# ihmcrobotics/mecano

Hardware: AMD Instinct MI355X
Metric: robot-configs/sec (RNEA+ABA), 30-DoF humanoid batch=4096 (higher is better)
Workload: dtype f64; 1 GPU; 30-DoF humanoid (SixDoF pelvis + 24 revolute), RNEA and ABA of every configuration per step, fp64, AoS [B][n] state; entry_point=mh_rnea_aba_f64, batch_per_gpu=4096, global_batch=4096, nq=31, nv=30, bodies=25, parallelism=dp1 (batch sharded, no data-path collective), kernel_variant=topo:b5c1e26c784c54fa, model_seed=43, state_seed=2342

## Files before the change

mecano_amd/csrc/mh_api.hip:

```cpp
#include "../../include/mecano_hip.h"
#include "mh_dfs_kernels.h"
#include "mh_split_kernels.h"
#include "mh_gravity_kernels.h"
#include "mh_response_kernels.h"
#include "mh_minv_kernels.h"
#include "mh_rnea_deriv_kernels.h"
#include "mh_params_kernels.h"

#include <dlfcn.h>
#include <spawn.h>
#include <sys/wait.h>
#include <unistd.h>
#include <cerrno>
extern char **environ;
#include <unistd.h>

#include <algorithm>
#include <functional>
#include <array>
#include <cmath>
#include <cstdarg>
#include <cstdio>
#include <cstdlib>
#include <cstring>
// ... 122 lines not shown
      T::operator=(v);
      return *this;
   }
};
}

struct SpecLib
{
   void *handle = nullptr;
   int (*launch)(int algo, int flags, const void *args, int grid, void *stream) = nullptr;
   long (*lds_bytes)(int algo, int flags, int nq, int nv) = nullptr;
   int (*aba_slots)(void) = nullptr;
   int (*supports)(int algo, int flags) = nullptr;
   int (*launch_fused)(int flags, const void *args, int waves, void *stream) = nullptr;
   long (*fused_lds_bytes)(int nq, int nv) = nullptr;
   int (*launch_crba)(int flags, const void *args, int grid, void *stream) = nullptr;
   int (*crba_packed)(int flags) = nullptr;
   int (*split_usable)(void) = nullptr;
   long (*split_lds_bytes)(int algo, int flags, int nq, int nv) = nullptr;
   int (*launch_split)(int algo, int flags, const void *args, int groups, void *stream) = nullptr;
   int (*crba_split_usable)(void) = nullptr;
   int (*launch_crba_split)(const void *args, int groups, int lanes_per_group, void *stream) = nullptr;
   int (*launch_rnea_crba)(const void *args, int rnea_groups, int crba_groups, int lanes_per_group, void *stream) = nullptr;
   long (*rnea_crba_lds_bytes)(int lanes_per_group, int nq, int nv) = nullptr;
   int (*launch_coriolis)(int flags, const void *args, int grid, void *stream) = nullptr;
   int (*launch_centroidal)(int flags, const void *args, int grid, void *stream) = nullptr;
   int (*launch_coriolis_parts)(int flags, const void *args, int grid, int parts, void *stream) = nullptr;
   int (*launch_centroidal_parts)(int flags, const void *args, int grid, int parts, void *stream) = nullptr;
   unsigned long long (*abi)(void) = nullptr;
   const char *(*sources_hash)(void) = nullptr;
   int (*zv_usable)(void) = nullptr;
   long (*zv_lds_bytes)(int nq, int nv) = nullptr;
   int (*launch_zv)(int flags, const void *args, void *taup, int *sync_flags, int *error, int epoch, int jobs, int same_l2, unsigned wait_ticks, void *stream) = nullptr;
   int (*zv_self_signal)(void) = nullptr;
   int (*zvb_usable)(void) = nullptr;
   int (*zvb_cs_rows)(void) = nullptr;
   long (*zvb_lds_bytes)(int which, int nq, int nv) = nullptr;
   int (*launch_zvb)(int flags, const void *args, void *taup, void *cs, long cs_stride, int groups, int which, void *stream) = nullptr;
   int (*zvf_usable)(void) = nullptr;
   int (*zvf_pair_usable)(void) = nullptr;
   int (*launch_zvf)(int flags, const void *args, int groups, void *stream) = nullptr;
   int (*launch_rnea_ahead)(int flags, const void *args, int groups, void *stream) = nullptr;
};
enum : int
{
   SPEC_IO_LDS = 1,
   SPEC_IDENT = 2,
   SPEC_ST_LDS = 4,
   SPEC_BODIES = 16,
   SPEC_OCC3 = 32
};

struct mh_model
{
   int n = 0, nq = 0, nv = 0, n_slots = 0;
   SpecLib spec;
   std::string topo_key;
   int device = 0;
   int cu_count = 256;
   std::vector<int> meta, dof_map, cfg_map;
   std::vector<int> engine_of;
   std::vector<double> consts;
   int *d_meta = nullptr, *d_dof = nullptr, *d_cfg = nullptr, *d_prog = nullptr;
   std::vector<int> prog;
   std::vector<int> prog_seq;
   int *d_prog_seq = nullptr;
// ... 278 lines not shown
}
std::mutex g_error_words_mutex;
std::vector<int *> g_error_words;
mh_status zv_check_error(mh_model *m)
{
   if (m->zv_error_host && *(volatile int *)m->zv_error_host != 0)
   {
      *(volatile int *)m->zv_error_host = 0;
      return fail(MH_ERR_HIP, "a bias-split forward dynamics launch gave up waiting for its bias rows (the accelerations of those configurations were written as NaN)");
   }
   return MH_OK;
}
mh_status check_all_error_words()
{
   std::lock_guard<std::mutex> lock(g_error_words_mutex);
   bool any = false;
   for (int *w : g_error_words)
      if (*(volatile int *)w != 0)
      {
         *(volatile int *)w = 0;
         any = true;
      }
   if (any)
      return fail(MH_ERR_HIP, "a bias-split forward dynamics launch gave up waiting for its bias rows (the accelerations of those configurations were written as NaN)");
   return MH_OK;
}
bool zv_self_signalling(const mh_model *m) { return m->ident_maps && m->spec.zv_self_signal && m->spec.zv_self_signal() != 0; }
mh_status zv_prepare(mh_model *m, int64_t B, hipStream_t stream)
{
   const size_t groups = (size_t)groups_of(B);
   mh_status st = ensure_bytes(m->zv_tau, groups * 64 * m->nv * sizeof(double));
   if (st != MH_OK)
      return st;
   if (zv_self_signalling(m) && m->zv_cols.bytes < groups * 64 * m->nv * sizeof(double))
   {
      st = ensure_bytes(m->zv_cols, std::max<size_t>(groups, 128) * 64 * m->nv * sizeof(double));
      if (st != MH_OK)
         return st;
      HIP_TRY(hipMemsetD32Async((hipDeviceptr_t)m->zv_cols.ptr, 0x7ff4a5a5, m->zv_cols.bytes / 4, stream));
   }
   if (m->zv_flags.bytes < groups * mh::ZV_SYNC_STRIDE * sizeof(int))
   {
      st = ensure_bytes(m->zv_flags, std::max<size_t>(groups, 1024) * mh::ZV_SYNC_STRIDE * sizeof(int));
      if (st != MH_OK)
         return st;
      HIP_TRY(hipMemsetAsync(m->zv_flags.ptr, 0, m->zv_flags.bytes, stream));
      m->zv_epoch = 0;
   }
   if (!m->zv_error_host)
   {
      HIP_TRY(hipHostMalloc((void **)&m->zv_error_host, 2 * sizeof(int), hipHostMallocMapped));
      m->zv_error_host[0] = m->zv_error_host[1] = 0;
      HIP_TRY(hipHostGetDevicePointer((void **)&m->zv_error_dev, m->zv_error_host, 0));
      std::lock_guard<std::mutex> lock(g_error_words_mutex);
      g_error_words.push_back(m->zv_error_host);
   }
   return MH_OK;
}
mh_status zv_launch(mh_model *m, mh::Args<double> &A, int jobs, hipStream_t stream, bool &done)
{
   done = false;
   mh_status st = zv_prepare(m, A.B, stream);
   if (st != MH_OK)
      return st;
   if (m->zv_epoch == 0x7fffffff)
   {
      HIP_TRY(hipDeviceSynchronize());
      HIP_TRY(hipMemsetAsync(m->zv_flags.ptr, 0, m->zv_flags.bytes, stream));
      m->zv_epoch = 0;
// ... 1140 lines not shown
      dir = e;
   std::string path = dir + "/libmecano_hip_topo_" + P.key + ".so";
   void *h = dlopen(path.c_str(), RTLD_NOW | RTLD_LOCAL);
   if (!h)
   {
      path = dir + "/libmecano_hip_topo_" + P.key + ".min.so";
      h = dlopen(path.c_str(), RTLD_NOW | RTLD_LOCAL);
   }
   if (!h)
      return;
   auto f_n = (int (*)(void))dlsym(h, "mh_spec_n");
   auto f_p = (const int *(*)(void))dlsym(h, "mh_spec_parents");
   auto f_t = (const int *(*)(void))dlsym(h, "mh_spec_types");
   SpecLib s;
   s.handle = h;
   s.launch = (decltype(s.launch))dlsym(h, "mh_spec_launch");
   s.lds_bytes = (decltype(s.lds_bytes))dlsym(h, "mh_spec_lds_bytes");
   s.aba_slots = (decltype(s.aba_slots))dlsym(h, "mh_spec_aba_slots");
   s.supports = (decltype(s.supports))dlsym(h, "mh_spec_supports");
   s.launch_fused = (decltype(s.launch_fused))dlsym(h, "mh_spec_launch_fused");
   s.fused_lds_bytes = (decltype(s.fused_lds_bytes))dlsym(h, "mh_spec_fused_lds_bytes");
   s.launch_crba = (decltype(s.launch_crba))dlsym(h, "mh_spec_launch_crba");
   s.crba_packed = (decltype(s.crba_packed))dlsym(h, "mh_spec_crba_packed");
   s.split_usable = (decltype(s.split_usable))dlsym(h, "mh_spec_split_usable");
   s.split_lds_bytes = (decltype(s.split_lds_bytes))dlsym(h, "mh_spec_split_lds_bytes");
   s.launch_split = (decltype(s.launch_split))dlsym(h, "mh_spec_launch_split");
   s.crba_split_usable = (decltype(s.crba_split_usable))dlsym(h, "mh_spec_crba_split_usable");
   s.launch_crba_split = (decltype(s.launch_crba_split))dlsym(h, "mh_spec_launch_crba_split");
   s.launch_rnea_crba = (decltype(s.launch_rnea_crba))dlsym(h, "mh_spec_launch_rnea_crba");
   s.zv_usable = (decltype(s.zv_usable))dlsym(h, "mh_spec_zv_usable");
   s.zv_lds_bytes = (decltype(s.zv_lds_bytes))dlsym(h, "mh_spec_zv_lds_bytes");
   s.launch_zv = (decltype(s.launch_zv))dlsym(h, "mh_spec_launch_zv");
   s.zv_self_signal = (decltype(s.zv_self_signal))dlsym(h, "mh_spec_zv_self_signal");
   s.zvb_usable = (decltype(s.zvb_usable))dlsym(h, "mh_spec_zvb_usable");
   s.zvb_cs_rows = (decltype(s.zvb_cs_rows))dlsym(h, "mh_spec_zvb_cs_rows");
   s.zvb_lds_bytes = (decltype(s.zvb_lds_bytes))dlsym(h, "mh_spec_zvb_lds_bytes");
   s.launch_zvb = (decltype(s.launch_zvb))dlsym(h, "mh_spec_launch_zvb");
   s.zvf_usable = (decltype(s.zvf_usable))dlsym(h, "mh_spec_zvf_usable");
   s.zvf_pair_usable = (decltype(s.zvf_pair_usable))dlsym(h, "mh_spec_zvf_pair_usable");
   s.launch_zvf = (decltype(s.launch_zvf))dlsym(h, "mh_spec_launch_zvf");
   s.launch_rnea_ahead = (decltype(s.launch_rnea_ahead))dlsym(h, "mh_spec_launch_rnea_ahead");
   s.rnea_crba_lds_bytes = (decltype(s.rnea_crba_lds_bytes))dlsym(h, "mh_spec_rnea_crba_lds_bytes");
   s.launch_coriolis = (decltype(s.launch_coriolis))dlsym(h, "mh_spec_launch_coriolis");
   s.launch_centroidal = (decltype(s.launch_centroidal))dlsym(h, "mh_spec_launch_centroidal");
   s.launch_coriolis_parts = (decltype(s.launch_coriolis_parts))dlsym(h, "mh_spec_launch_coriolis_parts");
   s.launch_centroidal_parts = (decltype(s.launch_centroidal_parts))dlsym(h, "mh_spec_launch_centroidal_parts");
   s.abi = (decltype(s.abi))dlsym(h, "mh_spec_abi");
   if (!s.abi || s.abi() != mh::spec_abi_stamp())
   {
      char note[256];
      snprintf(note, sizeof note, "generic (code object %s refused: built against another library version, ABI stamp %016llx, this library %016llx)",
               path.c_str(), s.abi ? s.abi() : 0ull, mh::spec_abi_stamp());
      m->variant = note;
      dlclose(h);
      return;
   }
   s.sources_hash = (decltype(s.sources_hash))dlsym(h, "mh_spec_sources_hash");
   if (!s.sources_hash || strcmp(s.sources_hash(), MH_STR_(MH_SPEC_SOURCES_HASH)) != 0)
   {
      char note[320];
      snprintf(note, sizeof note, "generic (code object %s refused: built from other kernel sources or flags, source hash %s, this library expects %s)",
               path.c_str(), s.sources_hash ? s.sources_hash() : "(none)", MH_STR_(MH_SPEC_SOURCES_HASH));
      m->variant = note;
      dlclose(h);
      return;
   }
// ... 2488 lines not shown
```

mecano_amd/csrc/mh_spec.hip:

```cpp
#include "mh_spec_kernels.h"
#include "mh_zv_kernels.h"

#include <algorithm>
#include <atomic>
#include <cstdlib>
#include <type_traits>

#ifndef MH_SPEC_PART
#define MH_SPEC_PART 0
#endif
#ifndef MH_TOPO_N
#error "MH_TOPO_N / MH_TOPO_PARENTS / MH_TOPO_TYPES must be defined"
#endif

namespace
{
struct TP
{
   static constexpr int N = MH_TOPO_N;
   static constexpr int parent[N] = {MH_TOPO_PARENTS};
   static constexpr int type[N] = {MH_TOPO_TYPES};
};
constexpr int kParents[TP::N] = {MH_TOPO_PARENTS};
constexpr int kTypes[TP::N] = {MH_TOPO_TYPES};
// ... 193 lines not shown
#else
      if constexpr (SPL::usable())
      {
         if (id && io && (algo == 0 || algo == 1))
         {
            static LdsAttr attr0, attr1;
            const size_t lds = (size_t)split_lds_bytes(algo, F_IO_LDS, A.m.nq, A.m.nv);
            if (algo == 0)
               return (int)launch_lds(&mh::spec_split_kernel<TP, double, 0, true, true, true>, A, groups, lds, attr0, s);
            return (int)launch_lds(&mh::spec_split_kernel<TP, double, 1, true, true, true>, A, groups, lds, attr1, s);
         }
      }
      return (int)hipErrorNotSupported;
#endif
   }
   if (id && io)
      return (int)go_split_algo<true, true>(algo, A, groups, s, occ3);
#ifdef MH_SPEC_MINIMAL
   return (int)hipErrorNotSupported;
#else
   if (id)
      return (int)go_split_algo<true, false>(algo, A, groups, s, occ3);
   if (io)
      return (int)go_split_algo<false, true>(algo, A, groups, s, occ3);
   return (int)go_split_algo<false, false>(algo, A, groups, s, occ3);
#endif
}
#endif
#if MH_SPEC_PART != 1
long mh_spec_zv_lds_bytes(int nq, int nv)
{
   if constexpr (!SPL::usable())
      return 0;
   const long inertia = (long)(SPL::n_limbs() * mh::ZV_XW + SPL::ZV_TRUNK_SLOTS + nq + 2 * nv) * 64 * (long)sizeof(double);
   return std::max(inertia, split_lds_bytes(0, F_IO_LDS, nq, nv) + (long)mh::zv_bias_extra_rows<TP>() * 64 * (long)sizeof(double));
}
int mh_spec_zv_usable(void) { return SPL::usable() ? 1 : 0; }
int mh_spec_zv_self_signal(void) { return MH_ZV_TWO_STAGE && MH_ZV_SELF_SIGNAL ? 1 : 0; }
#ifdef MH_ZV_PROBE
int mh_spec_zv_probe_read(void *dst, size_t bytes) { return (int)hipMemcpyFromSymbol(dst, HIP_SYMBOL(mh::zv_probe), bytes); }
int mh_spec_zv_probe_body_read(void *dst, size_t bytes) { return (int)hipMemcpyFromSymbol(dst, HIP_SYMBOL(mh::zv_probe_body), bytes); }
#endif
int mh_spec_launch_zv(int flags, const void *args, void *taup, int *sync_flags, int *error, int epoch, int jobs, int same_l2, unsigned wait_ticks, void *stream)
{
   if constexpr (SPL::usable())
   {
      const mh::Args<double> &A = *(const mh::Args<double> *)args;
      if (!(flags & F_IO_LDS) || (jobs != 2 && jobs != 3))
         return (int)hipErrorNotSupported;
      const size_t lds = (size_t)mh_spec_zv_lds_bytes(A.m.nq, A.m.nv);
      if (lds > 160 * 1024)
         return (int)hipErrorNotSupported;
      const long groups = (A.B + 63) / 64, padded = (groups + 7) / 8 * 8;
      const mh::ZvSync sy{sync_flags, error, epoch, jobs, same_l2 ? 1 : 0, wait_ticks};
      hipStream_t s = (hipStream_t)stream;
      if (A.q_next && (!(flags & F_IDENT) || jobs != 2 || !MH_ZV_TWO_STAGE))
         return (int)hipErrorNotSupported;
      if ((flags & F_IDENT) && A.q_next)
      {
         static LdsAttr attr_step;
         auto kern = &mh::spec_zv_kernel<TP, double, true, true>;
         if (const hipError_t e = ensure_lds_attr(reinterpret_cast<const void *>(kern), lds, attr_step); e != hipSuccess)
            return (int)e;
         hipLaunchKernelGGL(kern, dim3((unsigned)(padded * jobs)), dim3(256), lds, s, A.q, A.qd, A.in3b, A.B, jobs, A, (double *)taup, sy);
         return (int)hipGetLastError();
      }
      if (flags & F_IDENT)
      {
         static LdsAttr attr;
         auto kern = &mh::spec_zv_kernel<TP, double, true>;
         if (const hipError_t e = ensure_lds_attr(reinterpret_cast<const void *>(kern), lds, attr); e != hipSuccess)
// ... 355 lines not shown
```

mecano_amd/csrc/mh_zv_kernels.h:

```cpp
#pragma once
#include "mh_spec_kernels.h"

namespace mh
{
template <class TP>
struct ZvStore
{
   static constexpr int REG_SLOTS = Split<TP>::zv_reg_slots();
   static constexpr int kind(int j) { return Split<TP>::is_trunk(j) ? ST_LDS_KIND : ST_REG_KIND; }
   static constexpr int index(int j) { return Split<TP>::is_trunk(j) ? Split<TP>::zv_trunk_slot(j) : Split<TP>::zv_reg_slot(j); }
   static constexpr bool shared(int j) { return !Split<TP>::is_trunk(j); }
};
template <class TP>
struct ZvbStore
{
   using S = Split<TP>;
   static constexpr bool root_in_regs(int j) { return S::staged() && j == S::root(); }
   static constexpr int REG_SLOTS = S::zv_reg_slots() + (S::staged() ? Tree<TP>::zv_slots_of(S::root() < 0 ? 0 : S::root(), true) : 0);
   static constexpr int trunk_slot(int j)
   {
      int s = 0;
      for (int i = 0; i < j; i++)
         s += S::is_trunk(i) && !root_in_regs(i) ? Tree<TP>::zv_slots_of(i, false) : 0;
      return s;
// ... 477 lines not shown
            const SV<T> pa = pA + SV<T>{u * sa, u * sl};
            up = force_up(TYPE, jx, Xb, pa);
         }
      }
      else if constexpr (TYPE == JT_SIXDOF)
      {
         SV<T> tau;
         if constexpr (CX::csmode == 3)
            tau = SV<T>{V3<T>{zvf_tau_get1<TP, J, 0, CX, T>(cx), zvf_tau_get1<TP, J, 1, CX, T>(cx), zvf_tau_get1<TP, J, 2, CX, T>(cx)},
                        V3<T>{zvf_tau_get1<TP, J, 3, CX, T>(cx), zvf_tau_get1<TP, J, 4, CX, T>(cx), zvf_tau_get1<TP, J, 5, CX, T>(cx)}};
         else
            tau = spec_vec<TYPE, DO, 1, CX, T>(cx, true);
         const SV<T> x = spd6_solve(st_get_ldl<J, CX, T>(cx), tau - pA);
         cx.st.template put<J, RS + 0>(x.a.x), cx.st.template put<J, RS + 1>(x.a.y), cx.st.template put<J, RS + 2>(x.a.z);
         cx.st.template put<J, RS + 3>(x.l.x), cx.st.template put<J, RS + 4>(x.l.y), cx.st.template put<J, RS + 5>(x.l.z);
         if constexpr (HAS_PARENT)
         {
            const JX<T> jx = spec_joint<TYPE, CO, CX, T>(cx);
            up = force_up(TYPE, jx, load_xb_j<TP, J, T>(c), tau);
         }
      }
      else if constexpr (HAS_PARENT)
      {
         JX<T> jx;
         jx.c = T(1), jx.s = T(0), jx.d = T(0);
         up = force_up(TYPE, jx, load_xb_j<TP, J, T>(c), pA);
      }
      MH_BODY_FENCE();
      ZV_STAMP_TAIL(J, 1);
      return up;
   }
};

template <class TP, int J, typename T, class CX, int MODE = 0>
struct ZvOut
{
   template <int K>
   static MH_DEV void children(const CX &cx, const SV<T> &a)
   {
      if constexpr (K < Tree<TP>::n_children(J))
      {
         constexpr int C = Tree<TP>::child(J, K);
         if constexpr (MODE == 1 && !Split<TP>::is_trunk(C))
         {
            if (cx.wave == Split<TP>::owner(Split<TP>::limb_index(C)))
               ZvOut<TP, C, T, CX, 0>::run(cx, a);
         }
         else
            ZvOut<TP, C, T, CX, MODE>::run(cx, a);
         children<K + 1>(cx, a);
      }
   }
   static MH_DEV void run(const CX &cx, const SV<T> &ap)
   {
      MH_BODY_FENCE();
      constexpr int TYPE = TP::type[J];
      constexpr bool HAS_PARENT = TP::parent[J] >= 0;
      constexpr bool LEAF = Tree<TP>::n_children(J) == 0;
      constexpr int DO = Tree<TP>::dof_ofs(J), CO = Tree<TP>::cfg_ofs(J);
      constexpr int RS = Tree<TP>::zv_result_slot(J, CX::SPolicy::shared(J));
      ZV_STAMP_TAIL(J, 2);
      const T *cp = cx.C + J * MC_STRIDE;
      asm volatile("" : "+s"(cp));
      const CRef<T> c{cp};
      const V3<T> Z{T(0), T(0), T(0)};
      SV<T> a{Z, Z};
// ... 18 lines not shown
            a.a.z += qdd;
         else
            a.l.z += qdd;
      }
      else if constexpr (TYPE == JT_SIXDOF)
      {
         const SV<T> x{V3<T>{cx.st.template get<J, RS + 0>(), cx.st.template get<J, RS + 1>(), cx.st.template get<J, RS + 2>()},
                       V3<T>{cx.st.template get<J, RS + 3>(), cx.st.template get<J, RS + 4>(), cx.st.template get<J, RS + 5>()}};
         if (MODE == 0 || cx.wave == 0)
            spec_write<TYPE, DO, CX, T>(cx, x - a);
         a = x;
      }
      MH_BODY_FENCE();
      ZV_STAMP_TAIL(J, 3);
      if constexpr (!LEAF)
         children<0>(cx, a);
   }
};

template <class TP, typename T, class CX, int MODE, int K = 0>
MH_DEV void zv_roots_in(const CX &cx)
{
   if constexpr (K < Tree<TP>::n_children(-1))
   {
      (void)ZvIn<TP, Tree<TP>::child(-1, K), T, CX, MODE>::run(cx);
      zv_roots_in<TP, T, CX, MODE, K + 1>(cx);
   }
}
template <class TP, typename T, class CX, int K = 0>
MH_DEV void zv_roots_fold(const CX &cx)
{
   if constexpr (K < Tree<TP>::n_children(-1))
   {
      (void)ZvFold<TP, Tree<TP>::child(-1, K), T, CX, 1>::run(cx);
      zv_roots_fold<TP, T, CX, K + 1>(cx);
   }
}
template <class TP, typename T, class CX, int K = 0>
MH_DEV void zv_roots_out(const CX &cx)
{
   if constexpr (K < Tree<TP>::n_children(-1))
   {
      const V3<T> Z{T(0), T(0), T(0)};
      ZvOut<TP, Tree<TP>::child(-1, K), T, CX, 1>::run(cx, SV<T>{Z, Z});
      zv_roots_out<TP, T, CX, K + 1>(cx);
   }
}
template <class TP, int W, int K, int LATE, typename T, class CX>
MH_DEV void zv_limbs_in_of(const CX &cx)
{
   using S = Split<TP>;
   if constexpr (K < S::n_limbs())
   {
      if constexpr (S::owner(K) == W && (LATE < 0 || (S::is_late(K) ? 1 : 0) == LATE))
      {
         if constexpr (CX::csmode != 3 && !(CX::csmode == 0 && MH_ZV_PRE_WAVE))
            zv_pre<TP, S::limb_root(K), T, CX>(cx);
         x_put_ia<K, CX, T>(cx, ZvIn<TP, S::limb_root(K), T, CX, (LATE >= 0 && S::cut_limb(W) == K ? 3 : 0)>::run(cx));
      }
      zv_limbs_in_of<TP, W, K + 1, LATE, T, CX>(cx);
   }
}
template <class TP, int W, int I, typename T, class CX>
MH_DEV void zv_subtrunks_of(const CX &cx)
{
   using S = Split<TP>;
   if constexpr (I < S::n_sub())
// ... 255 lines not shown
{
   using S = Split<TP>;
   if constexpr (K < S::n_limbs())
   {
      if constexpr (S::owner(K) == W && ZvWalk<TP, true>::relayed(K))
      {
         const lds_ptr<T> flag = cx.xbase + (K * ZV_XW + ZV_RELAY_FLAG) * 64;
         while (__builtin_amdgcn_ballot_w64(__hip_atomic_load(flag, __ATOMIC_RELAXED, __HIP_MEMORY_SCOPE_WORKGROUP) == T(0)) != 0)
            __builtin_amdgcn_s_sleep(1);
         asm volatile("" ::: "memory");
         ZvOut<TP, S::limb_root(K), T, CX, 0>::run(cx, x_get6<K, ZV_XW, ZV_RELAY_A, CX, T>(cx));
      }
      zv_relay_out<TP, W, K + 1, T, CX>(cx);
   }
}
template <class TP, int W, int K, int LATE, typename T, class CX>
MH_DEV void zv_limbs_fold_sel(const CX &cx)
{
   using S = Split<TP>;
   if constexpr (K < S::n_limbs())
   {
      if constexpr (S::owner(K) == W && (LATE < 0 || (S::is_late(K) ? 1 : 0) == LATE))
         x_put6<K, CX::fold_xw, 0, CX, T>(cx, ZvFold<TP, S::limb_root(K), T, CX, 0>::run(cx));
      zv_limbs_fold_sel<TP, W, K + 1, LATE, T, CX>(cx);
   }
}
template <class TP, int W, int I, typename T, class CX>
MH_DEV void zv_subtrunks_fold_of(const CX &cx)
{
   using S = Split<TP>;
   if constexpr (I < S::n_sub())
   {
      constexpr int ST = S::sub_top(I);
      if constexpr (S::sub_owner(ST) == W)
         x_put6<S::sub_slot(ST), CX::fold_xw, 6, CX, T>(cx, ZvFold<TP, ST, T, CX, 1>::run(cx));
      zv_subtrunks_fold_of<TP, W, I + 1, T, CX>(cx);
   }
}
struct ZvNoHook
{
   MH_DEV void after_early() const {}
   MH_DEV void after_late() const {}
   MH_DEV void before_out() const {}
};
template <class TP, int W, typename T, class CX, class HOOK = ZvNoHook>
MH_DEV void zv_fold_out(const CX &cx, const HOOK &hook = HOOK())
{
   using S = Split<TP>;
   if constexpr (W < 4)
   {
      if (cx.wave == W)
      {
         if constexpr (S::staged())
         {
#ifdef MH_ZV_PROBE
            const long k = (long)cx.own;
#endif
            if constexpr (zv_relay<CX>::value)
               zv_relay_clear<TP, W, 0, T, CX>(cx);
            zv_limbs_fold_sel<TP, W, 0, 0, T, CX>(cx);
            hook.after_early();
            ZV_STAMP(1, 7);
            zv_fold_barrier<CX>();
            zv_limbs_fold_sel<TP, W, 0, 1, T, CX>(cx);
            hook.after_late();
            zv_subtrunks_fold_of<TP, W, 0, T, CX>(cx);
            ZV_STAMP(1, 8);
            zv_fold_barrier<CX>();
            (void)ZvFold<TP, S::root(), T, CX, 2>::run(cx);
            ZV_STAMP(1, 9);
         }
         else
         {
            zv_limbs_fold_sel<TP, W, 0, -1, T, CX>(cx);
            hook.after_early();
            zv_fold_barrier<CX>();
            hook.after_late();
            zv_roots_fold<TP, T, CX>(cx);
         }
         if constexpr (CX::csmode >= 2)
            zv_fold_barrier<CX>();
         hook.before_out();
         asm volatile("" ::: "memory");
         zv_roots_out_wave<TP, W, T, CX>(cx);
         if constexpr (zv_relay<CX>::value)
            zv_relay_out<TP, W, 0, T, CX>(cx);
      }
      else
         zv_fold_out<TP, W + 1, T, CX, HOOK>(cx, hook);
   }
}

template <typename T, int N, int NT>
MH_DEV void zv_stage_rows(lds_ptr<T> dst, const T *src, int rows)
{
   constexpr int U = (64 * N + NT - 1) / NT;
   T r[U];
   const int n = rows * N, t = threadIdx.x;
#pragma unroll
   for (int u = 0; u < U; u++)
      r[u] = t + NT * u < n ? src[t + NT * u] : T(0);
#pragma unroll
   for (int u = 0; u < U; u++)
      if (t + NT * u < 64 * N)
         dst[t + NT * u] = r[u];
}

struct ZvSync
// ... 176 lines not shown
   if (ok)
   {
      c.issue(src, lane);
      if (__builtin_amdgcn_ballot_w64(active && zv_cols_pending(c)) != 0)
      {
         const unsigned long long t0 = __builtin_amdgcn_s_memrealtime();
         for (;;)
         {
            __builtin_amdgcn_s_sleep(1);
            c.issue(src, lane);
            if (__builtin_amdgcn_ballot_w64(active && zv_cols_pending(c)) == 0)
               break;
            if (__builtin_amdgcn_s_memrealtime() - t0 > (unsigned long long)sy.wait_ticks)
            {
               ok = false;
               break;
            }
         }
      }
   }
   if (ok)
   {
      c.commit(row);
      c.reset(reset, lane);
   }
   else if ((threadIdx.x & 63) == 0)
   {
      __hip_atomic_store(sy.error, 1, __ATOMIC_RELAXED, __HIP_MEMORY_SCOPE_SYSTEM);
      __hip_atomic_store(sy.error + 1, 1, __ATOMIC_RELAXED, __HIP_MEMORY_SCOPE_SYSTEM);
      __hip_atomic_store(sy.flags + ZV_POISON_WORD, 1, __ATOMIC_RELAXED, __HIP_MEMORY_SCOPE_AGENT);
   }
   return ok;
}
template <class TP, typename T, int SHARE>
struct ZvPublish
{
   static constexpr bool mine(int d) { return SHARE < 0 ? ZvCols<TP>::trunk(d) : (!ZvCols<TP>::trunk(d) && ZvCols<TP>::limb_number(d) % 3 == SHARE); }
   static constexpr int count()
   {
      int n = 0;
      for (int d = 0; d < ZvCols<TP>::NV; d++)
         n += mine(d) ? 1 : 0;
      return n;
   }
   T r[count() > 0 ? count() : 1];
   template <int D = 0, int K = 0>
   MH_DEV void read(lds_ptr<T> row)
   {
      if constexpr (D < ZvCols<TP>::NV)
      {
         if constexpr (mine(D))
         {
            r[K] = row[D];
            read<D + 1, K + 1>(row);
         }
         else
            read<D + 1, K>(row);
      }
   }
   template <int D = 0, int K = 0>
   MH_DEV void read_minus(lds_ptr<T> tau_row, lds_ptr<T> row)
   {
      if constexpr (D < ZvCols<TP>::NV)
      {
         if constexpr (mine(D))
         {
// ... 57 lines not shown
   if (threadIdx.x == 0)
      zv_limb_waves = 0;
   ZV_STAMP(0, 0);
   RowRegs<T, MH_ZV_TAU_LATE ? Tree<TP>::total_dofs() : 1, 256> rtau;
   if constexpr (MH_ZV_TAU_LATE)
   {
      RowRegs<T, Tree<TP>::total_cfgs(), 256> rq;
      RowRegs<T, Tree<TP>::total_dofs(), 256> rd;
      rq.issue(A.q + cfg0 * nq, rows), rd.issue(A.qd + cfg0 * nv, rows), rtau.issue(A.in3 + cfg0 * nv, rows);
      rq.commit(lq), rd.commit(lqd);
      zv_lds_barrier();
   }
   else
   {
      wave_stage_in<T, Tree<TP>::total_cfgs(), Tree<TP>::total_dofs(), 256>(lq, lqd, lx, A.q + cfg0 * nq, A.qd + cfg0 * nv, A.in3 + cfg0 * nv, rows);
      __syncthreads();
   }
   CX cx;
   fill_ctx<T>(cx, A, active ? cfg0 + lane : cfg0);
   cx.coriolis = 1, cx.accel = 0;
   cx.lq = lq + lane * nq, cx.lqd = lqd + lane * nv, cx.lx = lx + lane * nv, cx.lo = cx.lx;
   cx.wave = wave;
   cx.xbase = lxc + lane;
   cx.st.lbase = lst + lane;
   cx.st.gbase = nullptr, cx.st.stride = 0, cx.st.lane = 0;
   ZV_STAMP(0, 1);
   if (active)
      split_rnea_limbs<TP, 0, T, CX>(cx);
   ZV_STAMP(0, 2);
   if constexpr (MH_ZV_TAU_LATE)
      rtau.commit(lt);
   __syncthreads();
   ZV_STAMP(0, 3);
   T *const dst = taup + k * 64 * nv;
   int *const flags = sy.flags + k * ZV_SYNC_STRIDE;
   if (wave == 0)
   {
      if (active)
         rnea_trunk_roots<TP, T, CX>(cx);
      ZV_STAMP(0, 4);
      if constexpr (MH_ZV_TAU_LATE)
         ZvPublish<TP, T, -1>::run_minus(dst, lt + lane * nv, lx + lane * nv, lane);
      else
         ZvPublish<TP, T, -1>::run(dst, lx + lane * nv, lane);
      ZV_STAMP(0, 5);
#ifdef MH_ZV_TEST_FLAG_BEFORE_DRAIN
      if (lane == 0)
         __hip_atomic_store(flags, sy.epoch, __ATOMIC_RELAXED, __HIP_MEMORY_SCOPE_AGENT);
#endif
      asm volatile("s_waitcnt vmcnt(0)" ::: "memory");
      ZV_STAMP(0, 6);
#if !defined(MH_ZV_TEST_FLAG_BEFORE_DRAIN) && !defined(MH_ZV_TEST_NO_FLAG)
      if (lane == 0)
         __hip_atomic_store(flags, sy.epoch, __ATOMIC_RELAXED, __HIP_MEMORY_SCOPE_AGENT);
#endif
      ZV_STAMP(0, 7);
   }
   else
   {
      ZV_STAMP(0, 4);
#if !(MH_ZV_SELF_SIGNAL && defined(MH_ZV_TEST_NO_FLAG))
      if constexpr (MH_ZV_TAU_LATE)
      {
         if (wave == 1)
            ZvPublish<TP, T, 0>::run_minus(dst, lt + lane * nv, lx + lane * nv, lane);
         else if (wave == 2)
            ZvPublish<TP, T, 1>::run_minus(dst, lt + lane * nv, lx + lane * nv, lane);
         else
// ... 166 lines not shown
   }
   __syncthreads();
   ZV_STAMP(1, 6);
   asm volatile("" ::: "memory");
   if (active)
      zv_fold_out<TP, 0, T, CX>(cx);
   ZV_STAMP(1, 10);
   if constexpr (!MH_ZV_DIRECT_OUT)
   {
      __syncthreads();
      wave_copy_out<T, 256>(A.out + cfg0 * nv, lres, rows * nv);
   }
   ZV_STAMP(1, 11);
}

MH_DEV bool zv_wait_word(const ZvSync &sy, const int *f)
{
   if (__hip_atomic_load(f, __ATOMIC_RELAXED, __HIP_MEMORY_SCOPE_AGENT) == sy.epoch)
      return true;
   const unsigned long long t0 = __builtin_amdgcn_s_memrealtime();
   for (;;)
   {
      __builtin_amdgcn_s_sleep(1);
      if (__hip_atomic_load(f, __ATOMIC_RELAXED, __HIP_MEMORY_SCOPE_AGENT) == sy.epoch)
         return true;
      if (__builtin_amdgcn_s_memrealtime() - t0 > (unsigned long long)sy.wait_ticks)
      {
         if ((threadIdx.x & 63) == 0)
            __hip_atomic_store(sy.error, 1, __ATOMIC_RELAXED, __HIP_MEMORY_SCOPE_SYSTEM);
         return false;
      }
   }
}
template <class TP, typename T, bool STEP>
MH_DEV void zv_aba_group2(const Args<T> &A, long k, lds_ptr<T> lds, const T *taup, const ZvSync &sy)
{
   using S = Split<TP>;
   using CX = ZvRelayCtx<Ctx<T, true, true, ZvStore<TP>, false, 0>>;
   const int wave = __builtin_amdgcn_readfirstlane((int)(threadIdx.x >> 6));
   const int lane = threadIdx.x & 63;
   constexpr int nq = Tree<TP>::total_cfgs(), nv = Tree<TP>::total_dofs();
   const lds_ptr<T> lxc = lds, lst = lxc + S::n_limbs() * ZV_XW * 64, lq = lst + S::ZV_TRUNK_SLOTS * 64, lx = lq + 64 * nq, lres = lx + 64 * nv;
   ZV_STAMP(1, 14);
   const long cfg0 = k * 64;
   const int rows = (int)(A.B - cfg0 < 64 ? A.B - cfg0 : 64);
   const bool active = lane < rows;
   __shared__ int zv_gave_up;
   if (threadIdx.x == 0)
      zv_gave_up = 0;
   ZV_STAMP(1, 0);
#if MH_ZV_SELF_SIGNAL
   const int poison = __hip_atomic_load(sy.flags + ZV_POISON_WORD, __ATOMIC_RELAXED, __HIP_MEMORY_SCOPE_AGENT);
#endif
   zv_stage_rows<T, Tree<TP>::total_cfgs(), 256>(lq, A.q + cfg0 * nq, rows);
   __syncthreads();
   ZV_STAMP(1, 1);
   CX cx;
   fill_ctx<T>(cx, A, active ? cfg0 + lane : cfg0);
   cx.lq = lq + lane * nq, cx.lqd = lq, cx.lx = lx + lane * nv, cx.lo = lres + lane * nv;
   cx.wave = wave;
   cx.xbase = lxc + lane;
   cx.st.lbase = lst + lane;
   cx.st.gbase = nullptr, cx.st.stride = 0, cx.st.lane = 0;
#ifdef MH_ZV_PROBE
   cx.own = (unsigned long long)k;
#endif
   if (active)
      zv_limbs_in<TP, 0, T, CX>(cx);
   ZV_STAMP(1, 2);
   __syncthreads();
   ZV_STAMP(1, 3);
   if (active)
      zv_roots_in<TP, T, CX, (S::staged() ? 2 : 1)>(cx);
   ZV_STAMP(1, 4);
   RowRegs<T, STEP ? Tree<TP>::total_dofs() : 1, 256> rqd;
   if constexpr (STEP)
      rqd.issue(A.qd + cfg0 * nv, rows);
   const T *const src = taup + k * 64 * nv;
   const int *const flags = sy.flags + k * ZV_SYNC_STRIDE;
   const lds_ptr<T> row = lx + lane * nv;
#if MH_ZV_SELF_SIGNAL
   bool seen;
   {
      T *const back = const_cast<T *>(src);
      if (wave == 0)
         seen = zv_take_cols<TP, T, 0>(sy, src, back, row, lane, active, poison);
      else if (wave == 1)
         seen = zv_take_cols<TP, T, 1>(sy, src, back, row, lane, active, poison);
      else if (wave == 2)
         seen = zv_take_cols<TP, T, 2>(sy, src, back, row, lane, active, poison);
      else
         seen = zv_take_cols<TP, T, 3>(sy, src, back, row, lane, active, poison);
   }
   ZV_STAMP(1, 5);
#else
   bool seen = zv_wait_word(sy, flags + 1);
   ZV_STAMP(1, 5);
   if (wave == 0)
   {
      ZvColRegs<TP, T, 0> c;
      c.issue(src, lane), c.commit(row);
   }
   else if (wave == 1)
   {
      ZvColRegs<TP, T, 1> c;
      c.issue(src, lane), c.commit(row);
   }
   else if (wave == 2)
   {
      ZvColRegs<TP, T, 2> c;
      c.issue(src, lane), c.commit(row);
   }
   else
   {
      ZvColRegs<TP, T, 3> c;
      c.issue(src, lane), c.commit(row);
   }
#endif
   const int b_first = __hip_atomic_load(flags, __ATOMIC_RELAXED, __HIP_MEMORY_SCOPE_AGENT);
   zv_lds_barrier();
   ZV_STAMP(1, 6);
   asm volatile("" ::: "memory");
   struct TrunkTau : ZvNoHook
   {
      mutable ZvColRegs<TP, T, -1> c;
      const ZvSync &sy;
      const int *flags;
      const T *src;
      lds_ptr<T> row;
      int lane, b_first;
      bool &seen;
      MH_DEV void after_early() const
      {
         if (b_first != sy.epoch)
            seen = zv_wait_word(sy, flags) && seen;
         c.issue(src, lane);
      }
      MH_DEV void after_late() const { c.commit(row); }
   };
   const TrunkTau trunk{{}, {}, sy, flags, src, row, lane, b_first, seen};
   if (active)
      zv_fold_out<TP, 0, T, CX>(cx, trunk);
   ZV_STAMP(1, 10);
   if (!seen && lane == 0)
      zv_gave_up = 1;
   __syncthreads();
   if (threadIdx.x == 0)
   {
      __hip_atomic_store(const_cast<int *>(flags), 0, __ATOMIC_RELAXED, __HIP_MEMORY_SCOPE_AGENT);
      __hip_atomic_store(const_cast<int *>(flags) + 1, 0, __ATOMIC_RELAXED, __HIP_MEMORY_SCOPE_AGENT);
   }
   if (zv_gave_up)
   {
      for (int i = threadIdx.x; i < rows * nv; i += 256)
         reinterpret_cast<unsigned long long *>(A.out)[cfg0 * nv + i] = 0x7ff8000000000000ull;
      if constexpr (STEP)
      {
         for (int i = threadIdx.x; i < rows * nq; i += 256)
            reinterpret_cast<unsigned long long *>(A.q_next)[cfg0 * nq + i] = 0x7ff8000000000000ull;
         for (int i = threadIdx.x; i < rows * nv; i += 256)
            reinterpret_cast<unsigned long long *>(A.qd_next)[cfg0 * nv + i] = 0x7ff8000000000000ull;
      }
      return;
   }
   if constexpr (STEP)
   {
      rqd.commit(lx);
      __syncthreads();
      if (active)
         integrate_rows<TP, 0, T>(wave, lq + lane * nq, lx + lane * nv, lres + lane * nv, A.dt, T(0.5) * A.dt * A.dt);
      __syncthreads();
      wave_copy_out<T, 256>(A.q_next + cfg0 * nq, lq, rows * nq);
      wave_copy_out<T, 256>(A.qd_next + cfg0 * nv, lx, rows * nv);
   }
   wave_copy_out<T, 256>(A.out + cfg0 * nv, lres, rows * nv);
   ZV_STAMP(1, 11);
}

#ifndef MH_ZV_KERNEL_ATTR
#define MH_ZV_KERNEL_ATTR
// ... 479 lines not shown
```

Before: 313.4 million configs/s.

## Stream trunk bias forces into the ABA fold via self-signalling columns

Adds a trunk-in-fold mode for the two-stage bias-split ABA kernel. The producer publishes extra per-limb and parked trunk force columns alongside tau, and the consumer folds them into its articulated-body pass (new ZvFoldZ) instead of waiting on a separate flag word and tau columns. Each wave polls its own share of sentinel-tagged columns and resets them. The aim is to drop the flag-based handoff and let consumer work overlap with producer completion, at the cost of more LDS, larger exchange buffers and extra per-body force arithmetic.

```diff
diff --git a/mecano_amd/csrc/mh_api.hip b/mecano_amd/csrc/mh_api.hip
--- a/mecano_amd/csrc/mh_api.hip
+++ b/mecano_amd/csrc/mh_api.hip
@@ -178,6 +178,7 @@
    int (*zv_usable)(void) = nullptr;
    long (*zv_lds_bytes)(int nq, int nv) = nullptr;
    int (*launch_zv)(int flags, const void *args, void *taup, int *sync_flags, int *error, int epoch, int jobs, int same_l2, unsigned wait_ticks, void *stream) = nullptr;
+   int (*zv_cols)(void) = nullptr;
    int (*zv_self_signal)(void) = nullptr;
    int (*zvb_usable)(void) = nullptr;
    int (*zvb_cs_rows)(void) = nullptr;
@@ -522,9 +523,10 @@
    mh_status st = ensure_bytes(m->zv_tau, groups * 64 * m->nv * sizeof(double));
    if (st != MH_OK)
       return st;
-   if (zv_self_signalling(m) && m->zv_cols.bytes < groups * 64 * m->nv * sizeof(double))
-   {
-      st = ensure_bytes(m->zv_cols, std::max<size_t>(groups, 128) * 64 * m->nv * sizeof(double));
+   const size_t cols = m->spec.zv_cols ? (size_t)std::max(m->spec.zv_cols(), m->nv) : (size_t)m->nv;
+   if (zv_self_signalling(m) && m->zv_cols.bytes < groups * 64 * cols * sizeof(double))
+   {
+      st = ensure_bytes(m->zv_cols, std::max<size_t>(groups, 128) * 64 * cols * sizeof(double));
       if (st != MH_OK)
          return st;
       HIP_TRY(hipMemsetD32Async((hipDeviceptr_t)m->zv_cols.ptr, 0x7ff4a5a5, m->zv_cols.bytes / 4, stream));
@@ -1731,6 +1733,7 @@
    s.zv_lds_bytes = (decltype(s.zv_lds_bytes))dlsym(h, "mh_spec_zv_lds_bytes");
    s.launch_zv = (decltype(s.launch_zv))dlsym(h, "mh_spec_launch_zv");
    s.zv_self_signal = (decltype(s.zv_self_signal))dlsym(h, "mh_spec_zv_self_signal");
+   s.zv_cols = (decltype(s.zv_cols))dlsym(h, "mh_spec_zv_cols");
    s.zvb_usable = (decltype(s.zvb_usable))dlsym(h, "mh_spec_zvb_usable");
    s.zvb_cs_rows = (decltype(s.zvb_cs_rows))dlsym(h, "mh_spec_zvb_cs_rows");
    s.zvb_lds_bytes = (decltype(s.zvb_lds_bytes))dlsym(h, "mh_spec_zvb_lds_bytes");
diff --git a/mecano_amd/csrc/mh_spec.hip b/mecano_amd/csrc/mh_spec.hip
--- a/mecano_amd/csrc/mh_spec.hip
+++ b/mecano_amd/csrc/mh_spec.hip
@@ -249,11 +249,12 @@
 {
    if constexpr (!SPL::usable())
       return 0;
-   const long inertia = (long)(SPL::n_limbs() * mh::ZV_XW + SPL::ZV_TRUNK_SLOTS + nq + 2 * nv) * 64 * (long)sizeof(double);
+   const long inertia = (long)(SPL::n_limbs() * mh::ZV_XW + SPL::ZV_TRUNK_SLOTS + nq + 2 * nv + (mh::ZvTif<TP>::on() ? mh::ZvTif<TP>::WIN : 0)) * 64 * (long)sizeof(double);
    return std::max(inertia, split_lds_bytes(0, F_IO_LDS, nq, nv) + (long)mh::zv_bias_extra_rows<TP>() * 64 * (long)sizeof(double));
 }
 int mh_spec_zv_usable(void) { return SPL::usable() ? 1 : 0; }
 int mh_spec_zv_self_signal(void) { return MH_ZV_TWO_STAGE && MH_ZV_SELF_SIGNAL ? 1 : 0; }
+int mh_spec_zv_cols(void) { return mh::ZvTif<TP>::NC; }
 #ifdef MH_ZV_PROBE
 int mh_spec_zv_probe_read(void *dst, size_t bytes) { return (int)hipMemcpyFromSymbol(dst, HIP_SYMBOL(mh::zv_probe), bytes); }
 int mh_spec_zv_probe_body_read(void *dst, size_t bytes) { return (int)hipMemcpyFromSymbol(dst, HIP_SYMBOL(mh::zv_probe_body), bytes); }
diff --git a/mecano_amd/csrc/mh_zv_kernels.h b/mecano_amd/csrc/mh_zv_kernels.h
--- a/mecano_amd/csrc/mh_zv_kernels.h
+++ b/mecano_amd/csrc/mh_zv_kernels.h
@@ -533,6 +533,194 @@
    }
 };
 
+#ifndef MH_ZV_TRUNK_IN_FOLD
+#define MH_ZV_TRUNK_IN_FOLD 1
+#endif
+#ifndef MH_ZV_TWO_STAGE
+#define MH_ZV_TWO_STAGE 1
+#endif
+#ifndef MH_ZV_SELF_SIGNAL
+#define MH_ZV_SELF_SIGNAL 1
+#endif
+#ifndef MH_ZV_TAU_LATE
+#define MH_ZV_TAU_LATE 0
+#endif
+template <class TP>
+struct ZvTif
+{
+   using S = Split<TP>;
+   static constexpr int NV = Tree<TP>::total_dofs(), NQ = Tree<TP>::total_cfgs();
+   static constexpr int NL = S::n_limbs(), NT = S::RNEA_TRUNK_SLOTS / 8;
+   static constexpr int WIN = 6 * (NL + NT);
+   static constexpr int limb_slot(int k) { return 6 * k; }
+   static constexpr int park_slot(int j) { return 6 * NL + 6 * (S::rnea_trunk_slot(j) / 8); }
+   static constexpr int lds_slots() { return NL * 21 + S::ZV_TRUNK_SLOTS + NQ + 2 * NV + WIN; }
+   static constexpr bool on()
+   {
+      return MH_ZV_TRUNK_IN_FOLD != 0 && MH_ZV_TWO_STAGE != 0 && MH_ZV_SELF_SIGNAL != 0 && MH_ZV_TAU_LATE == 0 && S::usable() && lds_slots() * 64 * 8 <= 160 * 1024;
+   }
+   static constexpr int NC = on() ? NV + WIN : NV;
+   struct Tab
+   {
+      bool input[NV + WIN + 1] = {};
+      int number[NV + WIN + 1] = {};
+      int share[4] = {};
+   };
+   static constexpr Tab make()
+   {
+      Tab t;
+      for (int j = 0; j < TP::N; j++)
+      {
+         const int d0 = Tree<TP>::dof_ofs(j), n = Tree<TP>::ndof(j);
+         for (int d = d0; d < d0 + n; d++)
+            t.input[d] = S::is_trunk(j);
+      }
+      int n = 0;
+      for (int d = 0; d < NV + WIN; d++)
+      {
+         if (d >= NV)
+            t.input[d] = true;
+         t.number[d] = n;
+         if (t.input[d])
+            t.share[n % 4]++, n++;
+      }
+      t.number[NV + WIN] = n;
+      return t;
+   }
+   static constexpr Tab TAB = make();
+   static constexpr bool trunk_input(int d) { return TAB.input[d]; }
+   static constexpr int input_number(int d) { return TAB.number[d]; }
+   static constexpr int SHARE_CAP = (TAB.number[NV + WIN] + 3) / 4;
+};
+template <class CXB, typename T>
+struct ZvTifCtx : CXB
+{
+   static constexpr bool trunk_in_fold = true;
+   lds_ptr<T> zin;
+};
+template <class CX, class = void>
+struct zv_tif_ctx
+{
+   static constexpr bool value = false;
+};
+template <class CX>
+struct zv_tif_ctx<CX, std::enable_if_t<CX::trunk_in_fold>>
+{
+   static constexpr bool value = true;
+};
+template <int S0, class CX, typename T>
+MH_DEV SV<T> zin_get6(const CX &cx)
+{
+   return SV<T>{V3<T>{cx.zin[(S0 + 0) * 64], cx.zin[(S0 + 1) * 64], cx.zin[(S0 + 2) * 64]},
+                V3<T>{cx.zin[(S0 + 3) * 64], cx.zin[(S0 + 4) * 64], cx.zin[(S0 + 5) * 64]}};
+}
+template <int S0, class CX, typename T>
+MH_DEV void zin_put6(const CX &cx, const SV<T> &w)
+{
+   cx.zin[(S0 + 0) * 64] = w.a.x, cx.zin[(S0 + 1) * 64] = w.a.y, cx.zin[(S0 + 2) * 64] = w.a.z;
+   cx.zin[(S0 + 3) * 64] = w.l.x, cx.zin[(S0 + 4) * 64] = w.l.y, cx.zin[(S0 + 5) * 64] = w.l.z;
+}
+template <class TP, int J, typename T, class CX, int MODE>
+struct ZvFoldZ
+{
+   using Z = ZvTif<TP>;
+   template <int K>
+   static MH_DEV void children(const CX &cx, SV<T> &pA, SV<T> &f)
+   {
+      if constexpr (K < Tree<TP>::n_children(J))
+      {
+         constexpr int C = Tree<TP>::child(J, K);
+         SV<T> c, fc;
+         if constexpr (!Split<TP>::is_trunk(C))
+         {
+            c = x_get6<Split<TP>::limb_index(C), CX::fold_xw, 0, CX, T>(cx);
+            fc = zin_get6<Z::limb_slot(Split<TP>::limb_index(C)), CX, T>(cx);
+         }
+         else if constexpr (MODE == 2)
+         {
+            c = x_get6<Split<TP>::sub_slot(C), CX::fold_xw, 6, CX, T>(cx);
+            fc = zin_get6<Z::park_slot(C), CX, T>(cx);
+         }
+         else
+            c = ZvFoldZ<TP, C, T, CX, MODE>::run(cx, fc);
+         if constexpr (K == 0)
+            pA = c;
+         else
+            pA = pA + c;
+         f = f + fc;
+         children<K + 1>(cx, pA, f);
+      }
+   }
+   static MH_DEV SV<T> run(const CX &cx, SV<T> &fup)
+   {
+      MH_BODY_FENCE();
+      constexpr int TYPE = TP::type[J];
+      constexpr bool HAS_PARENT = TP::parent[J] >= 0;
+      constexpr bool LEAF = Tree<TP>::n_children(J) == 0;
+      constexpr int DO = Tree<TP>::dof_ofs(J), CO = Tree<TP>::cfg_ofs(J);
+      constexpr int RS = Tree<TP>::zv_result_slot(J, CX::SPolicy::shared(J));
+      const V3<T> Z0{T(0), T(0), T(0)};
+      SV<T> pA{Z0, Z0};
+      SV<T> f = zin_get6<Z::park_slot(J), CX, T>(cx);
+      if constexpr (!LEAF)
+         children<0>(cx, pA, f);
+      MH_BODY_FENCE();
+      ZV_STAMP_TAIL(J, 0);
+      const T *cp = cx.C + J * MC_STRIDE;
+      asm volatile("" : "+s"(cp));
+      const CRef<T> c{cp};
+      SV<T> up{Z0, Z0};
+      fup = f;
+      if constexpr (TYPE == JT_REVOLUTE || TYPE == JT_PRISMATIC)
+      {
+         const T tau = cx.in3(DO) - (TYPE == JT_REVOLUTE ? f.a.z : f.l.z);
+         JX<T> jx;
+         jx.c = T(1), jx.s = T(0), jx.d = T(0);
+         if constexpr (TYPE == JT_REVOLUTE)
+            jx.c = cx.st.template get<J, 7>(), jx.s = cx.st.template get<J, 8>();
+         else if constexpr (HAS_PARENT)
+            jx.d = cx.q(CO);
+         const V3<T> sa{cx.st.template get<J, 0>(), cx.st.template get<J, 1>(), cx.st.template get<J, 2>()};
+         const V3<T> sl{cx.st.template get<J, 3>(), cx.st.template get<J, 4>(), cx.st.template get<J, 5>()};
+         const T dinv = cx.st.template get<J, 6>();
+         const T u = tau - (TYPE == JT_REVOLUTE ? pA.a.z : pA.l.z);
+         cx.st.template put<J, RS>(u * dinv);
+         if constexpr (HAS_PARENT)
+         {
+            const XF<T> Xb = load_xb_j<TP, J, T>(c);
+            const SV<T> pa = pA + SV<T>{u * sa, u * sl};
+            up = force_up(TYPE, jx, Xb, pa);
+            fup = force_up(TYPE, jx, Xb, f);
+         }
+      }
+      else if constexpr (TYPE == JT_SIXDOF)
+      {
+         const SV<T> tau = spec_vec<TYPE, DO, 1, CX, T>(cx, true) - f;
+         const SV<T> x = spd6_solve(st_get_ldl<J, CX, T>(cx), tau - pA);
+         cx.st.template put<J, RS + 0>(x.a.x), cx.st.template put<J, RS + 1>(x.a.y), cx.st.template put<J, RS + 2>(x.a.z);
+         cx.st.template put<J, RS + 3>(x.l.x), cx.st.template put<J, RS + 4>(x.l.y), cx.st.template put<J, RS + 5>(x.l.z);
+         if constexpr (HAS_PARENT)
+         {
+            const JX<T> jx = spec_joint<TYPE, CO, CX, T>(cx);
+            const XF<T> Xb = load_xb_j<TP, J, T>(c);
+            up = force_up(TYPE, jx, Xb, tau);
+            fup = force_up(TYPE, jx, Xb, f);
+         }
+      }
+      else if constexpr (HAS_PARENT)
+      {
+         JX<T> jx;
+         jx.c = T(1), jx.s = T(0), jx.d = T(0);
+         const XF<T> Xb = load_xb_j<TP, J, T>(c);
+         up = force_up(TYPE, jx, Xb, pA);
+         fup = force_up(TYPE, jx, Xb, f);
+      }
+      MH_BODY_FENCE();
+      ZV_STAMP_TAIL(J, 1);
+      return up;
+   }
+};
+
 template <class TP, int J, typename T, class CX, int MODE = 0>
 struct ZvOut
 {
@@ -617,7 +805,13 @@
 {
    if constexpr (K < Tree<TP>::n_children(-1))
    {
-      (void)ZvFold<TP, Tree<TP>::child(-1, K), T, CX, 1>::run(cx);
+      if constexpr (zv_tif_ctx<CX>::value)
+      {
+         SV<T> fup;
+         (void)ZvFoldZ<TP, Tree<TP>::child(-1, K), T, CX, 1>::run(cx, fup);
+      }
+      else
+         (void)ZvFold<TP, Tree<TP>::child(-1, K), T, CX, 1>::run(cx);
       zv_roots_fold<TP, T, CX, K + 1>(cx);
    }
 }
@@ -939,13 +1133,20 @@
    if constexpr (I < S::n_sub())
    {
       constexpr int ST = S::sub_top(I);
-      if constexpr (S::sub_owner(ST) == W)
+      if constexpr (S::sub_owner(ST) == W && zv_tif_ctx<CX>::value)
+      {
+         SV<T> fup;
+         x_put6<S::sub_slot(ST), CX::fold_xw, 6, CX, T>(cx, ZvFoldZ<TP, ST, T, CX, 1>::run(cx, fup));
+         zin_put6<ZvTif<TP>::park_slot(ST), CX, T>(cx, fup);
+      }
+      else if constexpr (S::sub_owner(ST) == W)
          x_put6<S::sub_slot(ST), CX::fold_xw, 6, CX, T>(cx, ZvFold<TP, ST, T, CX, 1>::run(cx));
       zv_subtrunks_fold_of<TP, W, I + 1, T, CX>(cx);
    }
 }
 struct ZvNoHook
 {
+   template <int W>
    MH_DEV void after_early() const {}
    MH_DEV void after_late() const {}
    MH_DEV void before_out() const {}
@@ -966,7 +1167,7 @@
             if constexpr (zv_relay<CX>::value)
                zv_relay_clear<TP, W, 0, T, CX>(cx);
             zv_limbs_fold_sel<TP, W, 0, 0, T, CX>(cx);
-            hook.after_early();
+            hook.template after_early<W>();
             ZV_STAMP(1, 7);
             zv_fold_barrier<CX>();
             zv_limbs_fold_sel<TP, W, 0, 1, T, CX>(cx);
@@ -974,13 +1175,19 @@
             zv_subtrunks_fold_of<TP, W, 0, T, CX>(cx);
             ZV_STAMP(1, 8);
             zv_fold_barrier<CX>();
-            (void)ZvFold<TP, S::root(), T, CX, 2>::run(cx);
+            if constexpr (zv_tif_ctx<CX>::value)
+            {
+               SV<T> fup;
+               (void)ZvFoldZ<TP, S::root(), T, CX, 2>::run(cx, fup);
+            }
+            else
+               (void)ZvFold<TP, S::root(), T, CX, 2>::run(cx);
             ZV_STAMP(1, 9);
          }
          else
          {
             zv_limbs_fold_sel<TP, W, 0, -1, T, CX>(cx);
-            hook.after_early();
+            hook.template after_early<W>();
             zv_fold_barrier<CX>();
             hook.after_late();
             zv_roots_fold<TP, T, CX>(cx);
@@ -1223,6 +1430,176 @@
    }
    return ok;
 }
+MH_DEV void zv_give_up(const ZvSync &sy)
+{
+   __hip_atomic_store(sy.error, 1, __ATOMIC_RELAXED, __HIP_MEMORY_SCOPE_SYSTEM);
+   __hip_atomic_store(sy.error + 1, 1, __ATOMIC_RELAXED, __HIP_MEMORY_SCOPE_SYSTEM);
+   __hip_atomic_store(sy.flags + ZV_POISON_WORD, 1, __ATOMIC_RELAXED, __HIP_MEMORY_SCOPE_AGENT);
+}
+template <class TP, typename T, int W>
+struct ZvTifCols
+{
+   using Z = ZvTif<TP>;
+   static constexpr int CAP = Z::SHARE_CAP;
+   static constexpr bool mine(int d) { return Z::trunk_input(d) && Z::input_number(d) % 4 == W; }
+   static constexpr int count() { return Z::TAB.share[W]; }
+   template <int D = 0, int K = 0>
+   static MH_DEV void issue(T (&r)[CAP], const T *src, int lane)
+   {
+      if constexpr (D < Z::NC)
+      {
+         if constexpr (mine(D))
+         {
+            r[K] = __hip_atomic_load(src + D * 64 + lane, __ATOMIC_RELAXED, __HIP_MEMORY_SCOPE_AGENT);
+            issue<D + 1, K + 1>(r, src, lane);
+         }
+         else
+            issue<D + 1, K>(r, src, lane);
+      }
+   }
+   static MH_DEV bool pending(const T (&r)[CAP])
+   {
+      constexpr int N = count();
+      bool p = false;
+#pragma unroll
+      for (int i = 0; i < N; i++)
+         p = p || zv_is_sentinel(r[i]);
+      return p;
+   }
+   template <int D = 0, int K = 0>
+   static MH_DEV void commit(const T (&r)[CAP], lds_ptr<T> row, lds_ptr<T> zin)
+   {
+      if constexpr (D < Z::NC)
+      {
+         if constexpr (mine(D))
+         {
+            if constexpr (D < Z::NV)
+               row[D] = r[K];
+            else
+               zin[(D - Z::NV) * 64] = r[K];
+            commit<D + 1, K + 1>(r, row, zin);
+         }
+         else
+            commit<D + 1, K>(r, row, zin);
+      }
+   }
+   template <int D = 0>
+   static MH_DEV void reset(T *dst, int lane)
+   {
+      if constexpr (D < Z::NC)
+      {
+         if constexpr (mine(D))
+            __hip_atomic_store(reinterpret_cast<unsigned long long *>(dst) + D * 64 + lane, ZV_SENTINEL, __ATOMIC_RELAXED, __HIP_MEMORY_SCOPE_AGENT);
+         reset<D + 1>(dst, lane);
+      }
+   }
+};
+template <class TP, typename T>
+struct ZvTrunkIn : ZvNoHook
+{
+   mutable T r[ZvTif<TP>::SHARE_CAP];
+   const ZvSync &sy;
+   const T *src;
+   lds_ptr<T> row, zin;
+   int lane;
+   bool &seen;
+   template <int W>
+   MH_DEV void request() const
+   {
+      ZvTifCols<TP, T, W>::issue(r, src, lane);
+   }
+   template <int W>
+   MH_DEV void after_early() const
+   {
+      using C = ZvTifCols<TP, T, W>;
+      if (!seen)
+         return;
+      if (__builtin_amdgcn_ballot_w64(C::pending(r)) != 0)
+      {
+         const unsigned long long t0 = __builtin_amdgcn_s_memrealtime();
+         for (;;)
+         {
+            __builtin_amdgcn_s_sleep(1);
+            C::issue(r, src, lane);
+            if (__builtin_amdgcn_ballot_w64(C::pending(r)) == 0)
+               break;
+            if (__builtin_amdgcn_s_memrealtime() - t0 > (unsigned long long)sy.wait_ticks)
+            {
+               seen = false;
+               break;
+            }
+         }
+      }
+      if (seen)
+      {
+         C::commit(r, row, zin);
+         C::reset(const_cast<T *>(src), lane);
+      }
+      else if ((threadIdx.x & 63) == 0)
+         zv_give_up(sy);
+   }
+};
+template <typename T>
+MH_DEV T zv_times_one(T x)
+{
+   if constexpr (sizeof(T) == 8)
+   {
+      T y;
+      asm volatile("v_mul_f64 %0, 1.0, %1" : "=v"(y) : "v"(x));
+      return y;
+   }
+   else
+      return x;
+}
+template <class TP, typename T, int SHARE>
+struct ZvTifPublish
+{
+   using Z = ZvTif<TP>;
+   static constexpr bool mine(int d) { return d % 4 == SHARE; }
+   static constexpr int count() { return (Z::NC - SHARE + 3) / 4; }
+   T r[count() > 0 ? count() : 1];
+   template <int D = 0, int K = 0>
+   MH_DEV void read(lds_ptr<T> row, lds_ptr<T> xc, lds_ptr<T> park)
+   {
+      if constexpr (D < Z::NC)
+      {
+         if constexpr (mine(D))
+         {
+            if constexpr (D < Z::NV && Z::trunk_input(D))
+               r[K] = zv_times_one(row[D]);
+            else if constexpr (D < Z::NV)
+               r[K] = row[D];
+            else if constexpr (D - Z::NV < 6 * Z::NL)
+               r[K] = xc[(D - Z::NV) * 64];
+            else
+               r[K] = park[(8 * ((D - Z::NV - 6 * Z::NL) / 6) + (D - Z::NV - 6 * Z::NL) % 6) * 64];
+            read<D + 1, K + 1>(row, xc, park);
+         }
+         else
+            read<D + 1, K>(row, xc, park);
+      }
+   }
+   template <int D = 0, int K = 0>
+   MH_DEV void store(T *dst, int lane) const
+   {
+      if constexpr (D < Z::NC)
+      {
+         if constexpr (mine(D))
+         {
+            __hip_atomic_store(dst + D * 64 + lane, r[K], __ATOMIC_RELAXED, __HIP_MEMORY_SCOPE_AGENT);
+            store<D + 1, K + 1>(dst, lane);
+         }
+         else
+            store<D + 1, K>(dst, lane);
+      }
+   }
+   static MH_DEV void run(T *dst, lds_ptr<T> row, lds_ptr<T> xc, lds_ptr<T> park, int lane)
+   {
+      ZvTifPublish p;
+      p.read(row, xc, park);
+      p.store(dst, lane);
+   }
+};
 template <class TP, typename T, int SHARE>
 struct ZvPublish
 {
@@ -1346,8 +1723,33 @@
       rtau.commit(lt);
    __syncthreads();
    ZV_STAMP(0, 3);
-   T *const dst = taup + k * 64 * nv;
+   T *const dst = taup + k * 64 * ZvTif<TP>::NC;
    int *const flags = sy.flags + k * ZV_SYNC_STRIDE;
+   if constexpr (ZvTif<TP>::on())
+   {
+      ZV_STAMP(0, 4);
+#ifndef MH_ZV_TEST_NO_FLAG
+      if (active)
+      {
+         const lds_ptr<T> row = lx + lane * nv, xc = lxc + lane, park = lst + lane;
+         if (wave == 0)
+            ZvTifPublish<TP, T, 0>::run(dst, row, xc, park, lane);
+         else if (wave == 1)
+            ZvTifPublish<TP, T, 1>::run(dst, row, xc, park, lane);
+         else if (wave == 2)
+            ZvTifPublish<TP, T, 2>::run(dst, row, xc, park, lane);
+         else
+            ZvTifPublish<TP, T, 3>::run(dst, row, xc, park, lane);
+      }
+#endif
+      ZV_STAMP(0, 5);
+#ifdef MH_ZV_TEST_FLAG_BEFORE_DRAIN
+      if (lane == 0)
+         __hip_atomic_store(flags, sy.epoch, __ATOMIC_RELAXED, __HIP_MEMORY_SCOPE_AGENT);
+#endif
+      ZV_STAMP(0, 7);
+      return;
+   }
    if (wave == 0)
    {
       if (active)
@@ -1580,15 +1982,37 @@
       }
    }
 }
+template <class TP, typename T>
+struct ZvTrunkTau : ZvNoHook
+{
+   mutable ZvColRegs<TP, T, -1> c;
+   const ZvSync &sy;
+   const int *flags;
+   const T *src;
+   lds_ptr<T> row;
+   int lane, b_first;
+   bool &seen;
+   template <int W>
+   MH_DEV void after_early() const
+   {
+      if (b_first != sy.epoch)
+         seen = zv_wait_word(sy, flags) && seen;
+      c.issue(src, lane);
+   }
+   MH_DEV void after_late() const { c.commit(row); }
+};
 template <class TP, typename T, bool STEP>
 MH_DEV void zv_aba_group2(const Args<T> &A, long k, lds_ptr<T> lds, const T *taup, const ZvSync &sy)
 {
    using S = Split<TP>;
-   using CX = ZvRelayCtx<Ctx<T, true, true, ZvStore<TP>, false, 0>>;
+   constexpr bool TIF = ZvTif<TP>::on();
+   using CXR = ZvRelayCtx<Ctx<T, true, true, ZvStore<TP>, false, 0>>;
+   using CX = std::conditional_t<TIF, ZvTifCtx<CXR, T>, CXR>;
    const int wave = __builtin_amdgcn_readfirstlane((int)(threadIdx.x >> 6));
    const int lane = threadIdx.x & 63;
    constexpr int nq = Tree<TP>::total_cfgs(), nv = Tree<TP>::total_dofs();
    const lds_ptr<T> lxc = lds, lst = lxc + S::n_limbs() * ZV_XW * 64, lq = lst + S::ZV_TRUNK_SLOTS * 64, lx = lq + 64 * nq, lres = lx + 64 * nv;
+   [[maybe_unused]] const lds_ptr<T> lzin = lres + 64 * nv;
    ZV_STAMP(1, 14);
    const long cfg0 = k * 64;
    const int rows = (int)(A.B - cfg0 < 64 ? A.B - cfg0 : 64);
@@ -1610,6 +2034,8 @@
    cx.xbase = lxc + lane;
    cx.st.lbase = lst + lane;
    cx.st.gbase = nullptr, cx.st.stride = 0, cx.st.lane = 0;
+   if constexpr (TIF)
+      cx.zin = lzin + lane;
 #ifdef MH_ZV_PROBE
    cx.own = (unsigned long long)k;
 #endif
@@ -1624,8 +2050,8 @@
    RowRegs<T, STEP ? Tree<TP>::total_dofs() : 1, 256> rqd;
    if constexpr (STEP)
       rqd.issue(A.qd + cfg0 * nv, rows);
-   const T *const src = taup + k * 64 * nv;
-   const int *const flags = sy.flags + k * ZV_SYNC_STRIDE;
+   const T *const src = taup + k * 64 * ZvTif<TP>::NC;
+   [[maybe_unused]] const int *const flags = sy.flags + k * ZV_SYNC_STRIDE;
    const lds_ptr<T> row = lx + lane * nv;
 #if MH_ZV_SELF_SIGNAL
    bool seen;
@@ -1665,35 +2091,41 @@
       c.issue(src, lane), c.commit(row);
    }
 #endif
-   const int b_first = __hip_atomic_load(flags, __ATOMIC_RELAXED, __HIP_MEMORY_SCOPE_AGENT);
-   zv_lds_barrier();
-   ZV_STAMP(1, 6);
-   asm volatile("" ::: "memory");
-   struct TrunkTau : ZvNoHook
-   {
-      mutable ZvColRegs<TP, T, -1> c;
-      const ZvSync &sy;
-      const int *flags;
-      const T *src;
-      lds_ptr<T> row;
-      int lane, b_first;
-      bool &seen;
-      MH_DEV void after_early() const
-      {
-         if (b_first != sy.epoch)
-            seen = zv_wait_word(sy, flags) && seen;
-         c.issue(src, lane);
-      }
-      MH_DEV void after_late() const { c.commit(row); }
-   };
-   const TrunkTau trunk{{}, {}, sy, flags, src, row, lane, b_first, seen};
-   if (active)
-      zv_fold_out<TP, 0, T, CX>(cx, trunk);
+   if constexpr (TIF)
+   {
+      const ZvTrunkIn<TP, T> trunk{{}, {}, sy, src, row, lzin + lane, lane, seen};
+      if (seen && active)
+      {
+         if (wave == 0)
+            trunk.template request<0>();
+         else if (wave == 1)
+            trunk.template request<1>();
+         else if (wave == 2)
+            trunk.template request<2>();
+         else
+            trunk.template request<3>();
+      }
+      zv_lds_barrier();
+      ZV_STAMP(1, 6);
+      asm volatile("" ::: "memory");
+      if (active)
+         zv_fold_out<TP, 0, T, CX>(cx, trunk);
+   }
+   else
+   {
+      const int b_first = __hip_atomic_load(flags, __ATOMIC_RELAXED, __HIP_MEMORY_SCOPE_AGENT);
+      zv_lds_barrier();
+      ZV_STAMP(1, 6);
+      asm volatile("" ::: "memory");
+      const ZvTrunkTau<TP, T> trunk{{}, {}, sy, flags, src, row, lane, b_first, seen};
+      if (active)
+         zv_fold_out<TP, 0, T, CX>(cx, trunk);
+   }
    ZV_STAMP(1, 10);
    if (!seen && lane == 0)
       zv_gave_up = 1;
    __syncthreads();
-   if (threadIdx.x == 0)
+   if (!(TIF && MH_ZV_SELF_SIGNAL) && threadIdx.x == 0)
    {
       __hip_atomic_store(const_cast<int *>(flags), 0, __ATOMIC_RELAXED, __HIP_MEMORY_SCOPE_AGENT);
       __hip_atomic_store(const_cast<int *>(flags) + 1, 0, __ATOMIC_RELAXED, __HIP_MEMORY_SCOPE_AGENT);
```

Measured after the change: 292.3 million configs/s. 6.7% lower.
